# bartn8/vppstereo

Hardware: AMD Instinct MI355X
Metric: Mdisparities/s (HxWxD / s) VPP+rSGM at 540x960xD=192 (higher is better)
Workload: dtype u16

## Files before the change

vppstereo_amd/csrc/vpp_kernels.hip:

```cpp
#include "vppx_internal.h"

#include <math.h>
#include <string.h>
#include <mutex>
#include <stdlib.h>

#define LG 992
#define RLCAP 8

struct HintRec {
    int x;
    float g;
    u32 base;
    u32 flags;
};

__host__ __device__ inline int vpp_bits_words(int W) { return (W + 63) / 64 + 2; }

struct VppK {
    int B, H, W, C;
    int n, direction, uniform, discard, interp, use_dist, use_bil;
    int wsize_m1;
    float c, c_occ, dmin, dmax;
    const float2 *range;
// ... 1569 lines not shown
}

u64 vpp_draws_upper_bound(const VppxVppParams &p, const VppGeom &g)
{
    const u64 n = (u64)((p.wsize - 1) / 2);
    const u64 per = p.uniform_color ? 1 : (2 * n + 1) * (2 * n + 1);
    u64 ub = (u64)g.H * g.W * g.C * per;
    ub = (ub + LG - 1) / LG * LG;
    return ub;
}

static Poly31 qoff_for(u64 rand_offset)
{
    static std::mutex m;
    static bool have0 = false;
    static Poly31 q0;
    Poly31 q;
    if (rand_offset == 0) {
        std::lock_guard<std::mutex> lk(m);
        if (!have0) { poly_pow_z(310, q0.c); have0 = true; }
        return q0;
    }
    poly_pow_z(rand_offset + 310, q.c);
    return q;
}

int vpp_launch(vppx_ctx *ctx, const VppxVppParams &p, const VppGeom &g, u8 *l, u8 *r, const float *gmap,
               const u8 *occ, const float *filled_g, int64_t *n_hints_dev, const u32 *seeds_dev, const u8 *r_orig)
{
    if (g.C < 1 || g.C > 4) { vppx_set_error("channels must be 1..4 (got %d)", g.C); return VPPX_E_INVALID_ARG; }
    if (p.wsize < 1 || p.wsize > 31) { vppx_set_error("wsize must be in 1..31 (got %d)", p.wsize); return VPPX_E_INVALID_ARG; }
    if (g.W > 32767 || g.H > 65535) {
        vppx_set_error("frames larger than 65535 x 32767 are not supported (got %d x %d)", g.H, g.W);
        return VPPX_E_UNSUPPORTED;
    }
    VppK k;
    k.B = g.B; k.H = g.H; k.W = g.W; k.C = g.C;
    k.n = (p.wsize - 1) / 2;
    k.wsize_m1 = p.wsize - 1;
    k.direction = p.direction != 0;
    k.uniform = p.uniform_color != 0;
    k.discard = p.discard_occluded != 0;
    k.interp = p.interpolate != 0;
    k.use_dist = p.use_distance_patch != 0;
    k.use_bil = (p.use_bilateral_patch != 0) && filled_g != nullptr;
    k.c = p.c; k.c_occ = p.c_occ; k.dmin = p.dmin; k.dmax = p.dmax;
    k.range = nullptr;
    k.inv_gamma = 1.0 / p.distance_gamma;
    k.l = l; k.r = r; k.r_src = r_orig ? r_orig : r; k.g = gmap; k.occ = occ; k.filled = filled_g;
    const size_t npx = (size_t)g.B * g.H * g.W;
    int rc;
    if ((rc = ws_get(ctx, WS_HINT_REC, npx, &k.rec))) return rc;
    if ((rc = ws_get(ctx, WS_HINT_DENSE, npx, &k.dense))) return rc;
    if ((rc = ws_get(ctx, WS_HINT_X, npx, &k.rng))) return rc;
    if ((rc = ws_get(ctx, WS_HINT_BITS, (size_t)g.B * g.H * vpp_bits_words(g.W), &k.bits))) return rc;
    k.rcnt = nullptr;
    k.lwork = nullptr;
    k.lwork_cnt = nullptr;
    k.rlist = nullptr;
    if ((rc = ws_get(ctx, WS_ROW_COUNT, (size_t)g.B * g.H, &k.row_count))) return rc;
    if ((rc = ws_get(ctx, WS_ROW_DRAWS, (size_t)g.B * g.H, &k.row_draws))) return rc;
    if ((rc = ws_get(ctx, WS_ROW_BASE, (size_t)g.B * g.H, &k.row_base))) return rc;
    if ((rc = ws_get(ctx, WS_FRAME_TOT, (size_t)g.B * 2, &k.frame_tot))) return rc;
    if (k.use_dist && p.per_frame_range) {
        float2 *range;
        if ((rc = ws_get(ctx, WS_HINT_RANGE, (size_t)g.B, &range))) return rc;
        hint_range_kernel<<<dim3(g.B), 1024, 0, ctx->stream>>>(gmap, (size_t)g.H * g.W, range);
        front_route_note(ctx, "hint_range");
        VPPX_CHECK_LAUNCH();
        k.range = range;
    }
    if (p.method == VPPX_METHOD_MAXDIST) {
        if (p.wsize_agg_x < 1 || p.wsize_agg_y < 1) { vppx_set_error("wsize_agg must be >= 1"); return VPPX_E_INVALID_ARG; }
        if ((rc = ws_get(ctx, WS_HINT_X, npx, &k.rng))) return rc;
        k.rnd = nullptr;
        k.rnd_cap = 0;
        k.uniform = 1;
        if (k.use_dist) compact_kernel<true><<<dim3((g.H + 3) / 4, g.B), 256, 0, ctx->stream>>>(k);
        else compact_kernel<false><<<dim3((g.H + 3) / 4, g.B), 256, 0, ctx->stream>>>(k);
        VPPX_CHECK_LAUNCH();
        front_route_note(ctx, "compact<%s>", k.use_dist ? "dist" : "plain");
        rowscan_kernel<<<dim3(g.B), 256, 0, ctx->stream>>>(k, (long long *)n_hints_dev);
        VPPX_CHECK_LAUNCH();
        front_route_note(ctx, "rowscan");
        stage_mark(ctx, ST_VPP_COMPACT);
        MdK m;
        m.k = k;
        m.k.uniform = p.uniform_color != 0;
        m.n_agg_x = (p.wsize_agg_x - 1) / 2;
        m.n_agg_y = (p.wsize_agg_y - 1) / 2;
        const int rad = k.n + m.n_agg_y;
        const size_t lds = (size_t)2 * (2 * rad + 1) * g.W;
        const size_t lds_wave = (size_t)2 * MD_RING * g.W;
        const int md = ctx->knobs.maxdist;
        if (md == 0 && k.direction && 2 * rad + 2 <= MD_RING && lds_wave <= 132 * 1024) {
            static bool attr_set[VPPX_MAX_DEVICES] = {};
            if (!attr_set[ctx->device & (VPPX_MAX_DEVICES - 1)]) {
                VPPX_HIP(hipFuncSetAttribute((const void *)maxdist_wave_kernel, hipFuncAttributeMaxDynamicSharedMemorySize, 132 * 1024));
                attr_set[ctx->device & (VPPX_MAX_DEVICES - 1)] = true;
            }
            maxdist_wave_kernel<<<dim3(g.B * g.C), 64 * MD_NW, lds_wave, ctx->stream>>>(m, rad);
            front_route_note(ctx, "maxdist_wave");
        } else if (lds <= 60 * 1024 && md != 2) {
            maxdist_lds_kernel<<<dim3(g.B * g.C), 64, lds, ctx->stream>>>(m, rad);
            front_route_note(ctx, "maxdist_lds");
        } else {
            maxdist_kernel<<<dim3(g.B * g.C), 64, 0, ctx->stream>>>(m);
            front_route_note(ctx, "maxdist_global");
        }
        VPPX_CHECK_LAUNCH();
        stage_mark(ctx, ST_VPP_APPLY);
        return 0;
    }
    const u64 cap = vpp_draws_upper_bound(p, g);
    u8 *rnd;
    if ((rc = ws_get(ctx, WS_RAND, (size_t)g.B * cap, &rnd))) return rc;
    k.rnd = rnd;
    k.rnd_cap = cap;
    const int nblk = (int)(cap / LG);
    const u32 *tab;
    if ((rc = ensure_rand_table(ctx, nblk, &tab))) return rc;
    if ((rc = ws_get(ctx, WS_LWORK, npx * 2, &k.lwork))) return rc;
    if ((rc = ws_get(ctx, WS_LWORK_CNT, (size_t)4, &k.lwork_cnt))) return rc;

    if (k.use_dist) compact_kernel<true><<<dim3((g.H + 3) / 4, g.B), 256, 0, ctx->stream>>>(k);
        else compact_kernel<false><<<dim3((g.H + 3) / 4, g.B), 256, 0, ctx->stream>>>(k);
    VPPX_CHECK_LAUNCH();
    front_route_note(ctx, "compact<%s>", k.use_dist ? "dist" : "plain");
    rowscan_kernel<<<dim3(g.B), 256, 0, ctx->stream>>>(k, (long long *)n_hints_dev);
    VPPX_CHECK_LAUNCH();
    front_route_note(ctx, "rowscan");
    stage_mark(ctx, ST_VPP_COMPACT);
    rand_kernel<<<dim3((nblk + 63) / 64, g.B), 64, 0, ctx->stream>>>(rnd, cap, k.frame_tot, seeds_dev, p.seed,
                                                                      qoff_for(p.rand_offset), tab, nblk);
    VPPX_CHECK_LAUNCH();
    front_route_note(ctx, "rand");
    stage_mark(ctx, ST_VPP_RAND);
    const int npairs = ((g.W + 255) / 256) * g.H;
    dim3 grid((unsigned)(npairs < 1024 ? npairs : 1024), g.B);
    if ((rc = ws_get(ctx, WS_RCNT, npx, &k.rcnt))) return rc;
    if ((rc = ws_get(ctx, WS_RLIST, npx * RLCAP, &k.rlist))) return rc;

    const bool split_early = (occ == nullptr) && ctx->stream2 != nullptr;
    const bool split_late = !split_early && r_orig != nullptr && r_orig != r && ctx->stream2 != nullptr;
    const bool split = split_early || split_late;
    const bool two_pass = occ != nullptr && !k.discard && k.n <= 3;
    if (!two_pass) k.lwork = nullptr;
    auto launch_l_hint = [&](hipStream_t st) {
        if (k.n > 3) return;
        const bool r4 = (long long)g.B * g.H >= 4 * 1024 && ctx->front_lds_budget >= 18 * 1024;
        const dim3 bg((unsigned)((g.W + 1023) / 1024), (unsigned)(r4 ? (g.H + 3) / 4 : g.H), (unsigned)g.B);
#define LB(NW) do { if (r4) apply_l_bits_kernel<NW, 4><<<bg, 256, 0, st>>>(k); else apply_l_bits_kernel<NW, 1><<<bg, 256, 0, st>>>(k); \
                    front_route_note(ctx, "l_bits<%d,%d>", NW, r4 ? 4 : 1); } while (0)
        switch (k.n) {
        case 0: LB(1); break;
        case 1: LB(3); break;
        case 2: LB(5); break;
        default: LB(7); break;
        }
#undef LB
    };
    auto launch_l_heavy = [&](hipStream_t st) {
        const dim3 hg((unsigned)(g.B * 512 < 32768 ? g.B * 512 : 32768));
        switch (k.n) {
#define LH(NW) do { apply_l_heavy_kernel<NW><<<hg, 64, 0, st>>>(k); front_route_note(ctx, "l_heavy<%d>", NW); } while (0)
        case 0: LH(1); break;
        case 1: LH(3); break;
        case 2: LH(5); break;
        default: LH(7); break;
#undef LH
        }
    };
    const bool wide_ids = g.W > 2048;
    int rr_nseg = wide_ids ? (g.W + 1023) / 1024 : 1;
    if (r_rows_lds((g.W + rr_nseg - 1) / rr_nseg, wide_ids) > ctx->front_lds_budget) {
        const int per_col = 4 + RLCAP * (wide_ids ? 4 : 2) + 4;
        const int sw_max = (int)((ctx->front_lds_budget > 2048 ? ctx->front_lds_budget - 512 : 1536) / per_col);
        rr_nseg = (g.W + sw_max - 1) / sw_max;
    }
    const int rr_sw = (g.W + rr_nseg - 1) / rr_nseg;
    const size_t rows_lds = r_rows_lds(rr_sw, wide_ids);
    const bool need_lists = occ != nullptr && !k.discard;
    if (!need_lists) k.rcnt = nullptr;
    auto launch_r_rows = [&](int mode) {
        if (wide_ids) r_rows_kernel<u32, 16, RR_NT><<<dim3(g.H * rr_nseg, g.B), RR_NT, rows_lds, ctx->stream>>>(k, mode, rr_sw);
        else r_rows_kernel<unsigned short, 11, RR_NT><<<dim3(g.H * rr_nseg, g.B), RR_NT, rows_lds, ctx->stream>>>(k, mode, rr_sw);
        front_route_note(ctx, "r_rows<%s,mode=%d,seg=%d>", wide_ids ? "u32" : "u16", mode, rr_nseg);
    };
    auto launch_l_wide = [&](hipStream_t st) {
        apply_l_wide_kernel<<<grid, 256, 0, st>>>(k);
        front_route_note(ctx, "l_wide");
    };
    hipStream_t ls = ctx->stream;
    if (split) {
        VPPX_HIP(hipEventRecord(ctx->ev_fork, ctx->stream));
        VPPX_HIP(hipStreamWaitEvent(ctx->stream2, ctx->ev_fork, 0));
        ls = ctx->stream2;
    }
    front_route_note(ctx, "vpp_order<%s,%s>", !need_lists ? "independent" : (split_late ? "late" : "inplace"), split ? "side" : "main");
    if (!need_lists) {
        launch_l_hint(ls);
        VPPX_CHECK_LAUNCH();
        if (k.n > 3) launch_l_wide(ls);
        VPPX_CHECK_LAUNCH();
        launch_r_rows(1);
        VPPX_CHECK_LAUNCH();
    } else if (split_late) {
        if (two_pass) {
            launch_l_hint(ls);
            VPPX_CHECK_LAUNCH();
        }
        launch_r_rows(3);
        VPPX_CHECK_LAUNCH();
        VPPX_HIP(hipEventRecord(ctx->ev_fork, ctx->stream));
        VPPX_HIP(hipStreamWaitEvent(ls, ctx->ev_fork, 0));
        if (two_pass) launch_l_heavy(ls);
        else launch_l_wide(ls);
        VPPX_CHECK_LAUNCH();
    } else {
        launch_r_rows(2);
        VPPX_CHECK_LAUNCH();
        launch_l_hint(ls);
        VPPX_CHECK_LAUNCH();
        if (two_pass) launch_l_heavy(ls);
        if (k.n > 3) launch_l_wide(ls);
        VPPX_CHECK_LAUNCH();
        launch_r_rows(1);
        VPPX_CHECK_LAUNCH();
    }
    if (split) {
        VPPX_HIP(hipEventRecord(ctx->ev_join, ctx->stream2));
        VPPX_HIP(hipStreamWaitEvent(ctx->stream, ctx->ev_join, 0));
    }
    stage_mark(ctx, ST_VPP_APPLY);
    return 0;
}

__global__ void __launch_bounds__(256) gray_ctx_kernel(const u8 *__restrict__ img, u8 *__restrict__ gray, size_t npix, int C)
{
    const size_t i = (size_t)blockIdx.x * blockDim.x + threadIdx.x;
    if (i >= npix) return;
    const u8 *s = img + i * C;
    gray[i] = C == 3 ? (u8)((s[2] * 9798u + s[1] * 19235u + s[0] * 3735u + 16384u) >> 15) : s[0];
}

__global__ void __launch_bounds__(256) bilateral_fill_kernel(const float *__restrict__ g, const u8 *__restrict__ gray,
                                                             float *__restrict__ out, int H, int W, int n, double inv2oxy,
                                                             double inv2oi, double th)
{
    const int x = blockIdx.x * blockDim.x + threadIdx.x;
    const int y = blockIdx.y, f = blockIdx.z;
    if (x >= W) return;
    const size_t base = (size_t)f * H * W;
    const int In = gray[base + (size_t)y * W + x];
    float cmap = 0.f;
    float aug = g[base + (size_t)y * W + x];
    for (int hy = max(0, y - n); hy <= min(H - 1, y + n); hy++)
        for (int hx = max(0, x - n); hx <= min(W - 1, x + n); hx++) {
            const float d_ref = g[base + (size_t)hy * W + hx];
            if (!(d_ref > 0)) continue;
            const int yw = y - hy, xw = x - hx;
            const long long di = (long long)In - (long long)gray[base + (size_t)hy * W + hx];
            const double a = __dadd_rn(__ddiv_rn((double)(yw * yw + xw * xw), inv2oxy), __ddiv_rn((double)(di * di), inv2oi));
            const double wgt = exp(-a);
            if ((double)cmap < wgt) {
                cmap = (float)wgt;
                aug = d_ref;
            }
        }
    out[base + (size_t)y * W + x] = ((double)cmap > th) ? aug : 0.f;
}

int vpp_launch_bilateral_fill(vppx_ctx *ctx, const VppxVppParams &p, const VppGeom &g, const u8 *left, const float *gmap,
                              float *filled_out)
{
    int rc;
    u8 *gray;
    const size_t npix = (size_t)g.B * g.H * g.W;
    if ((rc = ws_get(ctx, WS_GRAY_CTX, npix, &gray))) return rc;
    gray_ctx_kernel<<<dim3((unsigned)((npix + 255) / 256)), 256, 0, ctx->stream>>>(left, gray, npix, g.C);
    VPPX_CHECK_LAUNCH();
    front_route_note(ctx, "gray_ctx");
    dim3 grid((g.W + 255) / 256, g.H, g.B);
    bilateral_fill_kernel<<<grid, 256, 0, ctx->stream>>>(gmap, gray, filled_out, g.H, g.W, (p.wsize - 1) / 2,
                                                          2.0 * (p.bilateral_o_xy * p.bilateral_o_xy),
                                                          2.0 * (p.bilateral_o_i * p.bilateral_o_i), p.bilateral_th);
    VPPX_CHECK_LAUNCH();
    front_route_note(ctx, "bilateral_fill");
    return 0;
}

int vpp_launch_rand_stream(vppx_ctx *ctx, u32 seed, u64 offset, int64_t n, int32_t *out_dev)
{
    if (n <= 0) return 0;
    const int nblk = (int)((n + LG - 1) / LG);
    const u32 *tab;
    int rc;
    if ((rc = ensure_rand_table(ctx, nblk, &tab))) return rc;
    rand_full_kernel<<<dim3((nblk + 63) / 64), 64, 0, ctx->stream>>>(out_dev, (long long)n, seed, qoff_for(offset), tab, nblk);
    VPPX_CHECK_LAUNCH();
    return 0;
}

__global__ void __launch_bounds__(256) occ_warp4_kernel(const float4 *__restrict__ dmap, int *__restrict__ omap_bits, int H, int W)
{
    const int x4 = blockIdx.x * blockDim.x + threadIdx.x;
    const int y = blockIdx.y, f = blockIdx.z;
    if (4 * x4 >= W) return;
    const size_t row = ((size_t)f * H + y) * W;
    const float4 q = dmap[row / 4 + x4];
    const float v[4] = {q.x, q.y, q.z, q.w};
#pragma unroll
    for (int j = 0; j < 4; j++) {
        if (v[j] > 0) {
            const int xd = 4 * x4 + j - (int)rintf(v[j]);
            if (0 <= xd && xd <= W - 1) atomicMax(&omap_bits[row + xd], __float_as_int(v[j]));
        }
    }
}
__global__ void __launch_bounds__(256) occ_warp_kernel(const float *__restrict__ dmap, int *__restrict__ omap_bits, int H, int W)
{
    const int x = blockIdx.x * blockDim.x + threadIdx.x;
    const int y = blockIdx.y, f = blockIdx.z;
    if (x >= W) return;
    const size_t row = ((size_t)f * H + y) * W;
    const float v = dmap[row + x];
    if (v > 0) {
        const int xd = x - (int)rintf(v);
        if (0 <= xd && xd <= W - 1) atomicMax(&omap_bits[row + xd], __float_as_int(v));
    }
}
template <int NJ, int PT>
__global__ void __launch_bounds__(256) occ_test_kernel(const float *__restrict__ hints, const float *__restrict__ omap,
                                                       u8 *__restrict__ out, int *__restrict__ tmp, int H, int W, int rx,
                                                       int ry, double l, double g, double th, double th_filter)
{
    __shared__ int s_xd[256 * PT];
    __shared__ float s_v[256 * PT];
    __shared__ unsigned short s_px[256 * PT];
    __shared__ u8 s_cf[256 * PT];
    __shared__ int s_total;
    const int x0 = blockIdx.x * (256 * PT);
    const int y = blockIdx.y, f = blockIdx.z;
    const int t = threadIdx.x, lane = t & 63, wv = __builtin_amdgcn_readfirstlane(t >> 6);
    const float *om = omap + (size_t)f * H * W;
    const size_t row = ((size_t)f * H + y) * W;
    if (t == 0) s_total = 0;
    float v[PT], at[PT];
    int xd[PT];
#pragma unroll
    for (int u = 0; u < PT; u++) {
        const int x = x0 + 256 * u + t;
        v[u] = hints[row + min(x, W - 1)];
        if (x >= W) v[u] = 0.0f;
        s_cf[256 * u + t] = 0;
    }
#pragma unroll
    for (int u = 0; u < PT; u++) {
        xd[u] = x0 + 256 * u + t - (int)rintf(v[u]);
        at[u] = om[(size_t)y * W + min(max(xd[u], 0), W - 1)];
    }
    __syncthreads();
    bool owner[PT];
#pragma unroll
    for (int u = 0; u < PT; u++) {
        owner[u] = v[u] > 0 && 0 <= xd[u] && xd[u] <= W - 1 && at[u] == v[u];
        const unsigned long long bal = __builtin_amdgcn_ballot_w64(owner[u]);
        if (bal) {
            const int leader = __builtin_ctzll(bal);
            int base = 0;
            if (lane == leader) base = atomicAdd(&s_total, (int)__popcll(bal));
            base = __builtin_amdgcn_readlane(base, leader);
            if (owner[u]) {
                const int slot = base + (int)__builtin_amdgcn_mbcnt_hi((u32)(bal >> 32), __builtin_amdgcn_mbcnt_lo((u32)bal, 0u));
                s_xd[slot] = xd[u];
                s_v[slot] = v[u];
                s_px[slot] = (unsigned short)(256 * u + t);
            }
        }
    }
    __syncthreads();
    const int total = s_total;
    const int nyw = 2 * ry + 2, nwin = (2 * rx + 1) * nyw;
    if (NJ > 0) {
        int xwj[NJ > 0 ? NJ : 1], ycj[NJ > 0 ? NJ : 1];
        double wgj[NJ > 0 ? NJ : 1];
        bool inj[NJ > 0 ? NJ : 1];
#pragma unroll
        for (int j = 0; j < NJ; j++) {
            const int kpos = lane + 64 * j;
            xwj[j] = kpos / nyw - rx;
            const int yw = kpos % nyw - ry - 1;
            wgj[j] = __dmul_rn(l, __dadd_rn(__dmul_rn(g, (double)abs(xwj[j])), __dmul_rn(__dsub_rn(1.0, g), (double)abs(yw))));
            const int yc = y - yw;
            inj[j] = kpos < nwin && yc >= 0 && yc <= H - 1;
            ycj[j] = min(max(yc, 0), H - 1);
        }
        for (int e0 = 4 * wv; e0 < total; e0 += 16) {
            int xs[4];
            float ds[4], c[4][NJ > 0 ? NJ : 1];
#pragma unroll
            for (int i = 0; i < 4; i++) {
                const int e = e0 + i < total ? e0 + i : e0;
                xs[i] = s_xd[e];
                ds[i] = s_v[e];
            }
#pragma unroll
            for (int j = 0; j < NJ; j++) {
                const float *r = om + (size_t)ycj[j] * W;
#pragma unroll
                for (int i = 0; i < 4; i++) c[i][j] = r[min(max(xs[i] - xwj[j], 0), W - 1)];
            }
#pragma unroll
            for (int i = 0; i < 4; i++) {
                bool h = false;
#pragma unroll
                for (int j = 0; j < NJ; j++) {
                    const int xc = xs[i] - xwj[j];
                    if (inj[j] && xc >= 0 && xc <= W - 1 && c[i][j] > 0 && ds[i] < c[i][j])
                        h = h || (__dsub_rn((double)__fsub_rn(c[i][j], ds[i]), wgj[j]) > th);
                }
                if (__builtin_amdgcn_ballot_w64(h) != 0 && lane == 0 && e0 + i < total) s_cf[s_px[e0 + i]] = 1;
            }
        }
    } else {
        for (int e = wv; e < total; e += 4) {
            const int xs = s_xd[e];
            const float ds = s_v[e];
            bool hit = false;
            for (int kpos = lane; kpos < nwin; kpos += 64) {
                const int xw = kpos / nyw - rx, yw = kpos % nyw - ry - 1;
                const int yc = y - yw, xc = xs - xw;
                if (yc < 0 || yc > H - 1 || xc < 0 || xc > W - 1) continue;
                const float dc = om[(size_t)yc * W + xc];
                if (dc > 0 && ds < dc) {
                    const double tt = __dsub_rn((double)__fsub_rn(dc, ds),
                                                __dmul_rn(l, __dadd_rn(__dmul_rn(g, (double)abs(xw)),
                                                                       __dmul_rn(__dsub_rn(1.0, g), (double)abs(yw)))));
                    hit = hit || (tt > th);
                }
            }
            if (__builtin_amdgcn_ballot_w64(hit) != 0 && lane == 0) s_cf[s_px[e]] = 1;
        }
    }
    __syncthreads();
#pragma unroll
    for (int u = 0; u < PT; u++) {
        const int x = x0 + 256 * u + t;
        if (x >= W) continue;
        const int cf = s_cf[256 * u + t];
        const bool kept = owner[u] && !((double)cf > th_filter);
        out[row + x] = kept ? (u8)cf : (u8)1;
        if (tmp) tmp[row + x] = kept ? ((xd[u] << 1) | cf) : -1;
    }
}

__global__ void __launch_bounds__(256) occ_dmap_kernel(const int *__restrict__ tmp, const float *__restrict__ omap,
                                                       float *__restrict__ dmap_out, int H, int W)
{
    const int x = blockIdx.x * blockDim.x + threadIdx.x;
    const int y = blockIdx.y, f = blockIdx.z;
    if (x >= W) return;
    const size_t fb = (size_t)f * H * W;
    auto unwarped = [&](int yy, int xx) -> float {
        const size_t row = fb + (size_t)yy * W;
        const int t = tmp[row + xx];
        return t < 0 ? 0.0f : omap[row + (t >> 1)];
    };
    float u = unwarped(y, x);
    if (u == 0.0f) {
        const float nl = x > 0 ? unwarped(y, x - 1) : unwarped(y, W - 1);
        const float nr = x < W - 1 ? unwarped(y, x + 1) : (y < H - 1 ? unwarped(y + 1, 0) : 0.0f);
        if (nl > 0 && nr > 0 && fabs(__dsub_rn((double)nl, (double)nr)) < 1.0) {
            const double m = __ddiv_rn(__dsub_rn((double)nr, (double)nl), 2.0);
            const double q = __dsub_rn((double)nl, __dmul_rn(m, -1.0));
            u = (float)__dadd_rn(__dmul_rn(m, 0.0), q);
        }
    }
    dmap_out[fb + (size_t)y * W + x] = u;
}

int occ_launch(vppx_ctx *ctx, int B, int H, int W, const float *hints, int rx, int ry, double l, double g,
               double th_conf, double th_filter, float *omap, u8 *conf_out, float *dmap_out)
{
    const size_t n = (size_t)B * H * W;
    const bool small = ctx->front_lds_budget < 12 * 1024;
    dim3 grid((W + 255) / 256, H, B), grid_t((W + (small ? 511 : 1023)) / (small ? 512 : 1024), H, B);
    int *tmp = nullptr;
    if (dmap_out) {
        int rc = ws_get(ctx, WS_OCC_TMP, n, &tmp);
        if (rc) return rc;
    }
    VPPX_HIP(hipMemsetAsync(omap, 0, n * sizeof(float), ctx->stream));
    if (W % 4 == 0 && ((size_t)hints & 15) == 0) {
        occ_warp4_kernel<<<dim3((W / 4 + 255) / 256, H, B), 256, 0, ctx->stream>>>((const float4 *)hints, (int *)omap, H, W);
        front_route_note(ctx, "occ_warp4");
    } else {
        occ_warp_kernel<<<grid, 256, 0, ctx->stream>>>(hints, (int *)omap, H, W);
        front_route_note(ctx, "occ_warp");
    }
    VPPX_CHECK_LAUNCH();
    rx /= 2, ry /= 2;
    const long long nwin = (2LL * rx + 1) * (2LL * ry + 2);
#define OCC_TEST(NJ) do { if (small) occ_test_kernel<NJ, 2><<<grid_t, 256, 0, ctx->stream>>>(hints, omap, conf_out, tmp, H, W, rx, ry, l, g, th_conf, th_filter); \
                          else occ_test_kernel<NJ, 4><<<grid_t, 256, 0, ctx->stream>>>(hints, omap, conf_out, tmp, H, W, rx, ry, l, g, th_conf, th_filter); \
                          front_route_note(ctx, "occ_test<%d,%d>", NJ, small ? 2 : 4); } while (0)
    if (nwin <= 64) OCC_TEST(1);
    else if (nwin <= 128) OCC_TEST(2);
    else if (nwin <= 192) OCC_TEST(3);
    else if (nwin <= 256) OCC_TEST(4);
    else OCC_TEST(0);
#undef OCC_TEST
    VPPX_CHECK_LAUNCH();
    if (dmap_out) {
        occ_dmap_kernel<<<grid, 256, 0, ctx->stream>>>(tmp, omap, dmap_out, H, W);
        VPPX_CHECK_LAUNCH();
        front_route_note(ctx, "occ_dmap");
    }
    return 0;
}
```

Measured before the change: 429,400.

## Build occlusion warp map in LDS segments, drop global memset

The occlusion forward-warp kernels now give each block a 1024-pixel output segment held in shared memory. The block zeroes the segment, scans the source row from the segment start to the row end, and lands atomicMax updates in LDS instead of global memory. It then writes the whole segment out with vectorized stores, so the separate hipMemsetAsync over the occlusion map is no longer needed. In exchange, blocks re-read overlapping input tails (the full row remainder per segment), which adds redundant global reads when W exceeds one segment.

```diff
diff --git a/vppstereo_amd/csrc/vpp_kernels.hip b/vppstereo_amd/csrc/vpp_kernels.hip
--- a/vppstereo_amd/csrc/vpp_kernels.hip
+++ b/vppstereo_amd/csrc/vpp_kernels.hip
@@ -1895,33 +1895,61 @@
     return 0;
 }
 
+#define OCC_SEG 1024
+__device__ __forceinline__ void occ_seg_land(int *seg, int seg0, int segn, int x, float v)
+{
+    if (v > 0) {
+        const int xd = x - (int)rintf(v) - seg0;
+        if (0 <= xd && xd < segn) atomicMax(&seg[xd], __float_as_int(v));
+    }
+}
+__device__ __forceinline__ void occ_seg_store(const int *seg, int *__restrict__ out, int segn)
+{
+    const int t = threadIdx.x;
+    if (((size_t)out & 15) == 0) {
+        const int4 q = ((const int4 *)seg)[t];
+        if (4 * t + 3 < segn) ((int4 *)out)[t] = q;
+        else {
+            const int r[4] = {q.x, q.y, q.z, q.w};
+#pragma unroll
+            for (int j = 0; j < 4; j++)
+                if (4 * t + j < segn) out[4 * t + j] = r[j];
+        }
+    } else {
+#pragma unroll
+        for (int u = 0; u < OCC_SEG / 256; u++)
+            if (256 * u + t < segn) out[256 * u + t] = seg[256 * u + t];
+    }
+}
 __global__ void __launch_bounds__(256) occ_warp4_kernel(const float4 *__restrict__ dmap, int *__restrict__ omap_bits, int H, int W)
 {
-    const int x4 = blockIdx.x * blockDim.x + threadIdx.x;
-    const int y = blockIdx.y, f = blockIdx.z;
-    if (4 * x4 >= W) return;
+    __shared__ __attribute__((aligned(16))) int seg[OCC_SEG];
+    const int t = threadIdx.x, y = blockIdx.y, f = blockIdx.z;
+    const int seg0 = blockIdx.x * OCC_SEG, segn = min(OCC_SEG, W - seg0);
     const size_t row = ((size_t)f * H + y) * W;
-    const float4 q = dmap[row / 4 + x4];
-    const float v[4] = {q.x, q.y, q.z, q.w};
-#pragma unroll
-    for (int j = 0; j < 4; j++) {
-        if (v[j] > 0) {
-            const int xd = 4 * x4 + j - (int)rintf(v[j]);
-            if (0 <= xd && xd <= W - 1) atomicMax(&omap_bits[row + xd], __float_as_int(v[j]));
-        }
-    }
+    ((int4 *)seg)[t] = make_int4(0, 0, 0, 0);
+    __syncthreads();
+    for (int x4 = seg0 / 4 + t; 4 * x4 < W; x4 += 256) {
+        const float4 q = dmap[row / 4 + x4];
+        occ_seg_land(seg, seg0, segn, 4 * x4 + 0, q.x);
+        occ_seg_land(seg, seg0, segn, 4 * x4 + 1, q.y);
+        occ_seg_land(seg, seg0, segn, 4 * x4 + 2, q.z);
+        occ_seg_land(seg, seg0, segn, 4 * x4 + 3, q.w);
+    }
+    __syncthreads();
+    occ_seg_store(seg, omap_bits + row + seg0, segn);
 }
 __global__ void __launch_bounds__(256) occ_warp_kernel(const float *__restrict__ dmap, int *__restrict__ omap_bits, int H, int W)
 {
-    const int x = blockIdx.x * blockDim.x + threadIdx.x;
-    const int y = blockIdx.y, f = blockIdx.z;
-    if (x >= W) return;
+    __shared__ __attribute__((aligned(16))) int seg[OCC_SEG];
+    const int t = threadIdx.x, y = blockIdx.y, f = blockIdx.z;
+    const int seg0 = blockIdx.x * OCC_SEG, segn = min(OCC_SEG, W - seg0);
     const size_t row = ((size_t)f * H + y) * W;
-    const float v = dmap[row + x];
-    if (v > 0) {
-        const int xd = x - (int)rintf(v);
-        if (0 <= xd && xd <= W - 1) atomicMax(&omap_bits[row + xd], __float_as_int(v));
-    }
+    ((int4 *)seg)[t] = make_int4(0, 0, 0, 0);
+    __syncthreads();
+    for (int x = seg0 + t; x < W; x += 256) occ_seg_land(seg, seg0, segn, x, dmap[row + x]);
+    __syncthreads();
+    occ_seg_store(seg, omap_bits + row + seg0, segn);
 }
 template <int NJ, int PT>
 __global__ void __launch_bounds__(256) occ_test_kernel(const float *__restrict__ hints, const float *__restrict__ omap,
@@ -2084,12 +2112,12 @@
         int rc = ws_get(ctx, WS_OCC_TMP, n, &tmp);
         if (rc) return rc;
     }
-    VPPX_HIP(hipMemsetAsync(omap, 0, n * sizeof(float), ctx->stream));
+    const dim3 grid_w((W + OCC_SEG - 1) / OCC_SEG, H, B);
     if (W % 4 == 0 && ((size_t)hints & 15) == 0) {
-        occ_warp4_kernel<<<dim3((W / 4 + 255) / 256, H, B), 256, 0, ctx->stream>>>((const float4 *)hints, (int *)omap, H, W);
+        occ_warp4_kernel<<<grid_w, 256, 0, ctx->stream>>>((const float4 *)hints, (int *)omap, H, W);
         front_route_note(ctx, "occ_warp4");
     } else {
-        occ_warp_kernel<<<grid, 256, 0, ctx->stream>>>(hints, (int *)omap, H, W);
+        occ_warp_kernel<<<grid_w, 256, 0, ctx->stream>>>(hints, (int *)omap, H, W);
         front_route_note(ctx, "occ_warp");
     }
     VPPX_CHECK_LAUNCH();
```

Result: no change. 429,800 (median of 4 runs) (+0.1%).
